# LANL-Bioinformatics/FaQCs

Hardware: AMD Instinct MI355X
Metric: M reads/sec (paired 2x150bp) (higher is better)
Workload: dtype u8; 1 GPU; synthetic 100M-pair 2x150bp Q33 reads resident in HBM per GPU, BWA_plus -q 5 --min_L 50, 1 step = 1 pass (trim_lds + counter all-reduce); pairs_per_gpu=100000000, read_len=150, terminal_n_supplied=True

## Files before the change

### faqcs_amd/csrc/faqcs_capi.hip

```cpp
#include "faqcs_ctx.h"

static uint8_t na_to_bits_host(char c)
{
    switch (c) {
    case 'A': case 'a': return 1;  case 'C': case 'c': return 2;  case 'G': case 'g': return 4;
    case 'T': case 't': return 8;  case 'M': case 'm': return 3;  case 'R': case 'r': return 5;
    case 'S': case 's': return 6;  case 'V': case 'v': return 7;  case 'W': case 'w': return 9;
    case 'Y': case 'y': return 10; case 'H': case 'h': return 11; case 'K': case 'k': return 12;
    case 'D': case 'd': return 13; case 'B': case 'b': return 14; case 'N': case 'n': return 15;
    case '-': return 16;
    }
    return 0;
}

static void build_avgq(const faqcs_params &p, std::vector<int32_t> &avgq)
{
    const int N = FAQCS_TAB_LEN + 1;
    avgq.assign(N, 0);
    const volatile float avg = p.average_quality;
    if (!(avg > 0.0f)) return;
    for (int len = 1; len < N; ++len) {
        auto pass = [&](int V) {
            volatile float t = (float)(V + p.input_quality_offset * len) / (float)len;
            volatile float v = t - (float)p.input_quality_offset;
// ... 69 lines not shown
    for (auto &rs : c->rec) { HIPCHK(hipEventCreateWithFlags(&rs.trimmed, hipEventDisableTiming)); HIPCHK(hipEventCreateWithFlags(&rs.folded, hipEventDisableTiming)); }
    HIPCHK(hipEventCreateWithFlags(&c->copied, hipEventDisableTiming));
    for (auto &sl : c->slot) HIPCHK(hipEventCreateWithFlags(&sl.done, hipEventDisableTiming));
    for (auto &e : c->ticket_ev) HIPCHK(hipEventCreateWithFlags(&e, hipEventDisableTiming));
    faqcs_counters_layout(p->max_read_length, p->n_adapters, &c->lay);

    std::vector<uint32_t> lcthr, magic, basetab; std::vector<int32_t> avgq; std::vector<float> norm;
    build_tables(*p, lcthr, avgq, norm, magic, basetab);
    HIPCHK(upload(&c->d_lcthr, lcthr)); HIPCHK(upload(&c->d_avgq, avgq)); HIPCHK(upload(&c->d_norm, norm));
    HIPCHK(upload(&c->d_magic, magic)); HIPCHK(upload(&c->d_basetab, basetab));
    HIPCHK(hipMalloc((void **)&c->d_counters, c->lay.total * sizeof(uint64_t)));
    HIPCHK(hipMemset(c->d_counters, 0, c->lay.total * sizeof(uint64_t)));
    HIPCHK(hipMalloc((void **)&c->d_err, 256));
    HIPCHK(hipMemset(c->d_err, 0, 256));
    {
        const size_t dwords = (size_t)c->n_cu * FAQCS_PARTIAL_FLUSHES * FAQCS_PARTIAL_ROW + (size_t)c->n_cu;
        HIPCHK(hipMalloc((void **)&c->d_partials, dwords * sizeof(uint32_t)));
        HIPCHK(hipMemset(c->d_partials, 0, dwords * sizeof(uint32_t)));
    }

    if (p->n_adapters) {
        std::vector<uint8_t> bits; std::vector<uint32_t> start(1, 0);
        for (uint32_t j = 0; j < p->n_adapters; ++j) {
            const char *s = p->adapter_seq[j];
            const size_t L = strlen(s);
            if (L == 0 || L > FAQCS_MAX_ADAPTER_LENGTH)
                return fail(FAQCS_E_INVAL, "faqcs_create: adapter " + std::to_string(j) + " has " + std::to_string(L) + " bases, 1 ... " +
                                               std::to_string(FAQCS_MAX_ADAPTER_LENGTH) + " are supported");
            c->adapters.emplace_back(s);
            for (size_t k = 0; k < L; ++k) {
                const uint8_t b = na_to_bits_host(s[k]);
                if (!b) return fail(FAQCS_E_BASE, "seq_overlap.cpp:na_to_bits: Unknown base!");
                bits.push_back(b);
// ... 31 lines not shown
            HIPCHK(upload(&c->d_awstart_grp, wgrp));
        }
    }

    DevParams &d = c->dp;
    memset(&d, 0, sizeof(d));
    d.mode = p->mode; d.Q = p->quality; d.in_off = p->input_quality_offset; d.out_off = p->output_quality_offset;
    auto cap16 = [](uint32_t v) { return v > 65535u ? 65535u : v; };
    d.min_len = cap16(p->min_read_length); d.max_poly_n = cap16(p->max_num_poly_N); d.trim5 = cap16(p->trim_5); d.trim3 = cap16(p->trim_3);
    d.replace_q = p->replace_to_N_q; d.protect5 = p->protect_5; d.qc_only = p->qc_only;
    d.has_adapters = p->n_adapters ? 1 : 0; d.avgq_on = p->average_quality > 0.0f ? 1 : 0;
    d.R = p->max_read_length; d.n_adapters = p->n_adapters;
    d.lc_ratio = p->low_complexity_cutoff_ratio; d.avg_q = p->average_quality;
    if (const char *e = getenv("FAQCS_DBG")) d.dbg = (uint32_t)strtoul(e, nullptr, 0);
    d.lc_thr = c->d_lcthr; d.avgq_min_v = c->d_avgq; d.comp_norm = c->d_norm; d.div_magic = c->d_magic; d.base_tab = c->d_basetab;
    d.partials = c->d_partials;
    d.partial_rows = c->d_partials + (size_t)c->n_cu * FAQCS_PARTIAL_FLUSHES * FAQCS_PARTIAL_ROW;
    d.lay = c->lay;

    c->kmer_active = p->kmer_rarefaction ? 1 : 0;
    if (p->kmer_rarefaction) {
        uint64_t slots = p->kmer_table_slots ? p->kmer_table_slots : (1ull << 28);
        uint64_t pow2 = 1; while (pow2 < slots) pow2 <<= 1;
        if (pow2 < (uint64_t)KG_SLICE_MIN << 16) pow2 = (uint64_t)KG_SLICE_MIN << 16;
        if (pow2 > (uint64_t)KG_SLICE_MAX << 16) return fail(FAQCS_E_INVAL, "faqcs_create: kmer_table_slots above 2^32");
        c->kt.mask = pow2 - 1;
        { uint32_t lg = 0; while ((1ull << lg) < pow2) ++lg; if (lg > 46) return fail(FAQCS_E_INVAL, "faqcs_create: kmer_table_slots too large"); c->kt.shift = 62 - lg; }
        if (const char *e = getenv("FAQCS_KMER_DIRECT")) c->kg.direct = atoi(e) != 0;
        c->kt.ovf_mask = std::max<uint64_t>(pow2 >> 4, 1ull << 16) - 1;
        { const uint32_t lg = 62 - c->kt.shift;
          int f = (int)lg - 27; f = f < 0 ? 0 : (f > 3 ? 3 : f);
          if (const char *e = getenv("FAQCS_KMER_FINE_BITS")) { const int v = atoi(e); if (v >= 0 && v <= 3) f = v; }
          while (f > 0 && (pow2 >> (16 + f)) < 16) --f;
// ... 15 lines not shown
extern "C" void faqcs_destroy(faqcs_ctx *c)
{
    if (!c) return;
    (void)hipSetDevice(c->device);
    if (c->compute) (void)hipStreamSynchronize(c->compute);
    if (c->copy) (void)hipStreamSynchronize(c->copy);
    if (c->aux) (void)hipStreamSynchronize(c->aux);
    for (auto &t : c->timings) { (void)hipEventDestroy(t.a); (void)hipEventDestroy(t.b); (void)hipEventDestroy(t.p); (void)hipEventDestroy(t.k0); (void)hipEventDestroy(t.k1); }
    if (c->comm) comm_release(c->comm);
    if (c->comm_ev) (void)hipEventDestroy(c->comm_ev);
    c->emit.release(); c->parse.release(); c->render.release(); c->pair.release(); c->render_pair.release(); c->inflate.release(); c->bgzf_index.release(); c->deflate.release(); c->detect.release(); c->gunzip.release();
    if (c->ins_a) (void)hipEventDestroy(c->ins_a);
    if (c->ins_b) (void)hipEventDestroy(c->ins_b);
    for (int k = 0; k < 2; ++k) { if (c->fwd_free[k]) (void)hipEventDestroy(c->fwd_free[k]); if (c->fwd_copied[k]) (void)hipEventDestroy(c->fwd_copied[k]); c->fwd_items[k].release(); }
    void *ptrs[] = {c->d_lcthr, c->d_basetab, c->d_avgq, c->d_norm, c->d_magic, c->d_counters, c->d_err, c->d_partials, c->d_abits, c->d_astart, c->d_aplanes, c->d_awstart,
                    c->d_awstart_grp, c->kt.slots, c->kt.stats, c->kt.dirty, c->d_fold_claim, c->d_snaps, c->d_ob, c->d_tot_by_epoch, c->d_first_hist};
    for (void *q : ptrs) if (q) (void)hipFree(q);
    for (auto &sl : c->slot) { sl.seq.release(); sl.qual.release(); sl.tn.release(); sl.off.release(); if (sl.done) (void)hipEventDestroy(sl.done); }
    for (auto &e : c->ticket_ev) if (e) (void)hipEventDestroy(e);
    c->s_seg.release(); c->s_sl.release(); c->s_hit.release(); c->s_res.release(); c->s_astate.release(); c->s_amask.release();
    for (auto &rs : c->rec) { rs.pre.release(); rs.post.release(); if (rs.trimmed) (void)hipEventDestroy(rs.trimmed); if (rs.folded) (void)hipEventDestroy(rs.folded); }
    if (c->aux) (void)hipStreamDestroy(c->aux);
    c->ob_items.release(); c->ob_wave_count.release(); c->ob_wave_offset.release();
    { void *kg_ptrs[] = {c->kg.dev.l1, c->kg.dev.l2, c->kg.dev.cur1, c->kg.dev.cur2, c->kg.dev.run_epoch, c->kg.dev.first_hist, c->kg.dev.tot_by_epoch, c->kg.dev.dense, c->kg.dev.big, c->kg.dev.n_big, c->kg.dev.redo};
      for (void *q : kg_ptrs) if (q) (void)hipFree(q);
      c->kg.defer.release();
      c->ks.l1.release(); c->ks.spill.release(); c->ks.cur1.release(); c->ks.run_epoch.release(); c->ks.defer.release(); c->ks.scratch.release();
      for (auto &ev : c->kg.flush_ev) { (void)hipEventDestroy(ev.first); (void)hipEventDestroy(ev.second); } }
    if (c->copied) (void)hipEventDestroy(c->copied);
    if (c->compute) (void)hipStreamDestroy(c->compute);
    if (c->copy) (void)hipStreamDestroy(c->copy);
// ... 55 lines not shown
    G.mask_words = (s.max_len + 63) / 64;
    HIPCHK(c->s_astate.reserve(n)); HIPCHK(c->s_amask.reserve((size_t)n * G.mask_words));
    HIPCHK(hipMemsetAsync(c->s_astate.p, 0, (size_t)n * sizeof(uint4), c->compute));
    G.state = c->s_astate.p; G.mask = c->s_amask.p; G.gstart = c->d_astart;
    for (size_t k = 0; k < c->agroups.size(); ++k) {
        const faqcs_ctx::AdapterGroupHost &g = c->agroups[k];
        AdapterDev A{c->d_abits, c->d_astart + g.j0, c->d_aplanes + 4 * (size_t)g.w0, c->d_awstart_grp + g.j0 + k, g.n, c->match_rate,
                     g.longest, g.plane_dwords};
        G.j0 = g.j0; G.last = k + 1 == c->agroups.size() ? 1u : 0u;
        HIPCHK(launch(A, &G));
    }
    return 0;
}

static bool env_on(const char *name) { const char *e = getenv(name); return !e || atoi(e) != 0; }

static int enqueue_trim(faqcs_ctx *c, Timing &t, const Submission &s, const uint32_t *d_sl, const uint16_t *d_hit)
{
    const uint32_t n = s.n;
    HIPCHK(hipEventRecord(t.a, c->compute));
    const bool tail_on = env_on("FAQCS_TAIL_FOLD");
    const bool offer_fold = c->pending_fold >= 0 && !c->pending_wide && tail_on;
    DevParams dp = c->dp;
    dp.fold_n = offer_fold ? c->pending_n : 0u;
    static const bool lds_on = env_on("FAQCS_TRIM_LDS"), lds4_on = env_on("FAQCS_TRIM_LDS4"), lds16_on = env_on("FAQCS_TRIM_LDS16");
    const char *e_long = getenv("FAQCS_TRIM_LONG");
    const TrimPlan plan = trim_plan(trim_options(dp), s.max_len, n, c->n_cu, TrimSwitches{e_long && atoi(e_long) != 0, lds_on, lds4_on, lds16_on});
    const bool long_reads = plan.kernel == TrimKernel::trim_long;
    dp.wide_records = plan.wide_records;
    const int set = (int)(c->n_enqueued++ & 1);
    faqcs_ctx::RecSet &rs = c->rec[set];
    if (rs.used) { HIPCHK(hipStreamWaitEvent(c->compute, rs.folded, 0)); rs.used = false; }
    const size_t need = plan.records_needed;
    if (need > rs.pre.cap) { HIPCHK(hipStreamSynchronize(c->aux)); HIPCHK(hipStreamSynchronize(c->compute)); }
    HIPCHK(rs.pre.reserve(need)); HIPCHK(rs.post.reserve(need));
    if (offer_fold) {
        const faqcs_ctx::RecSet &ps = c->rec[c->pending_fold];
        if (!c->d_fold_claim) HIPCHK(hipMalloc((void **)&c->d_fold_claim, 8));
        HIPCHK(hipMemsetAsync(c->d_fold_claim, 0, 8, c->compute));
        dp.fold_pre = ps.pre.p; dp.fold_post = ps.post.p; dp.fold_claim = c->d_fold_claim;
        dp.fold_dst_pre = c->d_counters + c->lay.pre_comp; dp.fold_dst_post = c->d_counters + c->lay.post_comp;
    }
    const TrimArgs a{s.seq, s.qual, s.off, n, s.max_len, d_sl, d_hit, s.tn, s.res, rs.pre.p, rs.post.p, c->d_counters, c->d_err, c->n_cu, c->compute};
    HIPCHK(long_reads ? faqcs_launch_trim_long(plan, dp, a)
                      : plan.kernel == TrimKernel::trim_lds ? faqcs_launch_trim_lds(plan, dp, a) : faqcs_launch_trim_filter_accumulate(plan, dp, a));
    HIPCHK(hipEventRecord(t.b, c->compute));
    c->trim_kernel = trim_kernel_name(plan.kernel);
    if (c->pending_fold >= 0) {
        if (!plan.folds_tail) {
            faqcs_ctx::RecSet &ps = c->rec[c->pending_fold];
            HIPCHK(hipStreamWaitEvent(c->aux, ps.trimmed, 0));
            HIPCHK(faqcs_launch_composition(ps.pre.p, ps.post.p, c->pending_n, c->pending_wide, c->d_norm, c->d_counters + c->lay.pre_comp,
                                            c->d_counters + c->lay.post_comp, c->n_cu, c->aux));
            HIPCHK(hipEventRecord(ps.folded, c->aux));
            ps.used = true;
        }
        c->pending_fold = -1;
    }
    static const bool no_comp = [] { const char *e = getenv("FAQCS_DIAG_NO_COMPOSITION"); return e && atoi(e) != 0; }();
    if (!(c->dp.dbg & 1u) && !long_reads && !no_comp) {
        HIPCHK(hipEventRecord(rs.trimmed, c->compute));
// ... 121 lines not shown
    if (!d_results) { HIPCHK(c->s_res.reserve((size_t)n + 1)); d_results = c->s_res.p; }
    return enqueue(c, b->seq, b->qual, b->offset, n, max_len, b->segment_start, b->n_segments, d_results, b->terminal_n);
}

extern "C" int faqcs_terminal_n_flags(int device_id, const uint8_t *d_seq, const uint32_t *d_offset, uint32_t n_reads, uint8_t *d_flags)
{
    if (!d_seq || !d_offset || !d_flags) return fail(FAQCS_E_INVAL, "null argument");
    if (device_id >= 0) HIPCHK(hipSetDevice(device_id));
    HIPCHK(faqcs_launch_terminal_n_flags(d_seq, d_offset, n_reads, d_flags, nullptr));
    HIPCHK(hipDeviceSynchronize());
    return 0;
}

int fold_pending_now(faqcs_ctx *c)
{
    if (c->pending_fold < 0) return 0;
    faqcs_ctx::RecSet &ps = c->rec[c->pending_fold];
    HIPCHK(faqcs_launch_composition(ps.pre.p, ps.post.p, c->pending_n, c->pending_wide, c->d_norm, c->d_counters + c->lay.pre_comp,
                                    c->d_counters + c->lay.post_comp, c->n_cu, c->compute));
    c->pending_fold = -1;
    return 0;
}

extern "C" int faqcs_sync(faqcs_ctx *c)
{
    if (!c) return fail(FAQCS_E_INVAL, "null ctx");
    HIPCHK(hipSetDevice(c->device));
    HIPCHK(hipStreamSynchronize(c->copy));
    if (int rc = fold_pending_now(c)) return rc;
    HIPCHK(hipStreamSynchronize(c->compute));
// ... 56 lines not shown
}

extern "C" int faqcs_finish(faqcs_ctx *c, uint64_t *counters, uint64_t n_u64)
{
    if (!c || !counters || n_u64 < c->lay.total) return fail(FAQCS_E_INVAL, "faqcs_finish: counter buffer too small");
    if (int rc = faqcs_sync(c)) return rc;
    HIPCHK(hipMemcpy(counters, c->d_counters, c->lay.total * sizeof(uint64_t), hipMemcpyDeviceToHost));
    return 0;
}

extern "C" int faqcs_reset_counters(faqcs_ctx *c)
{
    if (!c) return fail(FAQCS_E_INVAL, "null ctx");
    HIPCHK(hipSetDevice(c->device));
    c->pending_fold = -1;
    HIPCHK(hipStreamSynchronize(c->aux));
    HIPCHK(hipMemsetAsync(c->d_counters, 0, c->lay.total * sizeof(uint64_t), c->compute));
    return 0;
}

static int synth_fill_impl(int device_id, uint8_t *d_seq, uint8_t *d_qual, uint32_t *d_offset, uint32_t n_reads, uint32_t L,
                           uint64_t seed, uint64_t first_read, float adapter_frac, uint64_t genome_len)
{
    if (device_id >= 0) HIPCHK(hipSetDevice(device_id));
    if ((uint64_t)n_reads * L + L > 0xffffffffull) return fail(FAQCS_E_INVAL, "faqcs_synth_fill: arena exceeds 32-bit offsets");
    const char *at = getenv("FAQCS_SYNTH_AT");
    HIPCHK(faqcs_launch_synth(d_seq, d_qual, d_offset, n_reads, L, seed, first_read, adapter_frac, genome_len, at ? (float)atof(at) : -1.0f, nullptr));
    HIPCHK(hipDeviceSynchronize());
    return 0;
}
// ... 47 lines not shown
```

### faqcs_amd/csrc/faqcs_ctx.h

```cpp
#pragma once
#include <hip/hip_runtime.h>

#include <algorithm>
#include <cmath>
#include <cstdio>
#include <cstdlib>
#include <cstring>
#include <map>
#include <memory>
#include <string>
#include <vector>

#include "faqcs_dev.h"
#include "faqcs_host.h"
#include "faqcs_kmer.h"
#include "faqcs_skm.h"

struct AdapterDev {
    const uint8_t *bits;
    const uint32_t *start, *planes, *wstart;
    uint32_t n_adapters;
    float match_rate;
    uint32_t longest, plane_dwords;
};
hipError_t faqcs_launch_trim_lds(const TrimPlan &plan, const DevParams &P, const TrimArgs &a);
hipError_t faqcs_launch_trim_filter_accumulate(const TrimPlan &plan, const DevParams &P, const TrimArgs &a);
hipError_t faqcs_launch_trim_long(const TrimPlan &plan, const DevParams &P, const TrimArgs &a);
hipError_t faqcs_launch_terminal_n_flags(const uint8_t *seq, const uint32_t *off, uint32_t n_reads, uint8_t *flags, hipStream_t st);
hipError_t faqcs_launch_composition(const unsigned long long *rec_pre, const unsigned long long *rec_post, uint32_t n, bool wide,
                                    const float *comp_norm, uint64_t *dst_pre, uint64_t *dst_post, int n_cu, hipStream_t st);
hipError_t faqcs_launch_adapter(const AdapterDev &A, const AdapterGroup *G, const uint8_t *seq, const uint32_t *off, uint32_t n_reads,
                                uint32_t max_len, const uint32_t *seg_start, uint32_t n_segments, uint32_t *ad_sl,
                                uint16_t *ad_hit, uint64_t *adapter_stats, uint32_t *err, uint32_t dbg, int n_cu, hipStream_t st);
hipError_t faqcs_launch_synth(uint8_t *d_seq, uint8_t *d_qual, uint32_t *d_offset, uint32_t n_reads, uint32_t L,
                              uint64_t seed, uint64_t first_read, float adapter_frac, uint64_t genome_len, float at_frac, hipStream_t st);

size_t faqcs_emit_scratch_bytes(uint32_t n_reads);
hipError_t faqcs_launch_emit_scan(const uint8_t *seq, const uint32_t *off, const uint8_t *tn, uint32_t n_reads, const faqcs_read_result *res,
                                  const uint8_t *keep, const faqcs_emit_out *out, void *scratch, hipStream_t st);
hipError_t faqcs_launch_emit_gather(const uint8_t *seq, const uint8_t *qual, uint32_t n_reads, const faqcs_emit_out *out, const void *scratch,
// ... 128 lines not shown
    PackStage parse;
    PackStage render;
    PackStage pair;
    PackStage render_pair;
    PackStage inflate;
    PackStage bgzf_index;
    PackStage deflate;
    GunzipStage gunzip;
    PackStage detect;
    struct RecSet { DevBuf<unsigned long long> pre, post; hipEvent_t trimmed = nullptr, folded = nullptr; bool used = false; };
    RecSet rec[2];
    uint64_t n_enqueued = 0;
    int pending_fold = -1;
    uint32_t pending_n = 0;
    bool pending_wide = false;
    uint32_t *d_fold_claim = nullptr;
    hipStream_t aux = nullptr;
    uint64_t total_number = 0;
    int kmer_active = 0;
    std::vector<faqcs_rarefaction> points;
    struct PendingPoint { size_t point_index; size_t snap_index; };
    std::vector<PendingPoint> pending;
    KmerTable kt{nullptr, 0, nullptr, 0};
    bool partitioned = false;
    uint32_t part_rank = 0, part_world = 1, n_epochs = 0;
    std::vector<uint32_t> seg_epoch;
    DevBuf<ulonglong2> ob_items;
    bool ob_fresh = false;
    DevBuf<uint32_t> ob_wave_count;
    DevBuf<unsigned long long> ob_wave_offset;
    unsigned long long *d_ob = nullptr;
// ... 62 lines not shown
```

### faqcs_amd/csrc/faqcs_dev.h

```cpp
#pragma once
#include <hip/hip_runtime.h>
#include <stdint.h>

#include "../../include/faqcs_mi.h"
#include "faqcs_trim_plan.h"

#define FAQCS_WAVE 64
#define FAQCS_TAB_LEN FAQCS_FAST_READ_LENGTH

struct DevParams {
    int32_t mode, Q, in_off, out_off;
    uint32_t min_len, max_poly_n, trim5, trim3, replace_q;
    uint32_t protect5, qc_only, has_adapters, avgq_on;
    uint32_t R;
    uint32_t n_adapters;
    uint32_t dbg;
    uint32_t wide_records;
    float lc_ratio, avg_q;
    const uint32_t *lc_thr;
    const int32_t  *avgq_min_v;
    const uint32_t *div_magic;
    const float    *comp_norm;
    const uint32_t *base_tab;
    uint32_t *partials;
    uint32_t *partial_rows;
    faqcs_layout lay;
    const unsigned long long *fold_pre, *fold_post;
    uint32_t fold_n;
    uint32_t *fold_claim;
    uint64_t *fold_dst_pre, *fold_dst_post;
};

#define FAQCS_ADAPTER_GROUP 64
#define FAQCS_ADAPTER_TPL_CAP 4096
#define FAQCS_ADAPTER_SINGLE_LENGTH 8192

struct AdapterGroup {
    uint4 *state;
    uint64_t *mask;
    const uint32_t *gstart;
    uint32_t j0;
    uint32_t mask_words;
    uint32_t last;
};

enum { FAQCS_PARTIAL_ROW = 16896 };

struct TrimArgs {
    const uint8_t *seq, *qual;
    const uint32_t *off;
    uint32_t n_reads, max_len;
    const uint32_t *ad_sl;
    const uint16_t *ad_hit;
    const uint8_t *tn_flags;
    faqcs_read_result *out;
    unsigned long long *rec_pre, *rec_post;
    uint64_t *counters;
    uint32_t *err;
    int n_cu;
    hipStream_t st;
// ... 211 lines not shown
```

### faqcs_amd/csrc/faqcs_trim_common.h

```cpp
#pragma once
#include "faqcs_dev.h"

#include <stdlib.h>

static inline hipError_t ensure_dynamic_lds(const void *kernel, size_t bytes, unsigned long long &done)
{
    int dev = 0;
    hipError_t e = hipGetDevice(&dev);
    if (e != hipSuccess) return e;
    const unsigned long long bit = 1ull << (dev & 63);
    if (__atomic_load_n(&done, __ATOMIC_ACQUIRE) & bit) return hipSuccess;
    e = hipFuncSetAttribute(kernel, hipFuncAttributeMaxDynamicSharedMemorySize, (int)bytes);
    if (e == hipSuccess) __atomic_fetch_or(&done, bit, __ATOMIC_RELEASE);
    return e;
}

namespace {

template <int D> struct __attribute__((packed, aligned(1))) PackedBytes { uint32_t w[D]; };

__device__ __forceinline__ int med3i(int x, int lo, int hi) { return x < lo ? lo : (x > hi ? hi : x); }

template <int C> __device__ __forceinline__ uint32_t range_mask(int lo, int hi, int pbase)
{
// ... 501 lines not shown
        }
        if (dirty) {
            __syncthreads();
            for (int d = tid; d < ND; d += NT) {
                const uint32_t v = tab[d];
                if (v) {
                    tab[d] = 0;
                    if (v & 0xffffu) atomicAdd((unsigned long long *)(dst + 2 * d), (unsigned long long)(v & 0xffffu));
                    if (v >> 16) atomicAdd((unsigned long long *)(dst + 2 * d + 1), (unsigned long long)(v >> 16));
                }
            }
            __syncthreads();
        }
    }
}
#endif
```

### faqcs_amd/csrc/faqcs_trim_lds_kernel.hip

```cpp
#include "faqcs_trim_common.h"

#include <stdlib.h>
#include <type_traits>

#ifndef FAQCS_LDS_SUM_UNROLL
#define FAQCS_LDS_SUM_UNROLL 4
#endif
#ifndef FAQCS_LDS_SA_UNROLL
#define FAQCS_LDS_SA_UNROLL 2
#endif

namespace {

typedef uint32_t LdsPair2 __attribute__((ext_vector_type(2)));
typedef const __attribute__((address_space(3))) LdsPair2 *lds_u2c_ptr;
typedef __attribute__((address_space(3))) uint8_t *lds_u8_mut;
typedef const __attribute__((address_space(3))) uint8_t *lds_u8_ptr;
struct __attribute__((packed, aligned(1))) U32u { uint32_t w; };
typedef const __attribute__((address_space(3))) U32u *lds_u32u_ptr;

__device__ __forceinline__ uint32_t lds_ld(uint32_t byte_offset) { return *(lds_u32_ptr)(size_t)byte_offset; }
__device__ __forceinline__ uint32_t lds_ld_any(uint32_t byte_offset)
{
    const uint32_t a4 = byte_offset & ~3u;
// ... 158 lines not shown
__device__ __noinline__ void flush_block_partial(uint32_t *smem, uint32_t *__restrict__ row, const int tid)
{
    using Cfg = RowCfg<C, LPR, lds_wq(C, LPR)>;
    constexpr int N4 = (Cfg::N_ZERO + 3) / 4;
    static_assert(N4 * 4 <= FAQCS_PARTIAL_ROW, "partial-sum row");
    __syncthreads();
    for (int i = tid; i < N4; i += NW * 64) {
        const uint4 v = reinterpret_cast<const uint4 *>(smem)[i];
        reinterpret_cast<uint4 *>(row)[i] = v;
        if (4 * i + 3 < Cfg::N_ZERO) reinterpret_cast<uint4 *>(smem)[i] = make_uint4(0u, 0u, 0u, 0u);
        else for (int k = 4 * i; k < Cfg::N_ZERO; ++k) smem[k] = 0u;
    }
    __syncthreads();
}

template <int C, int LPR>
__global__ __launch_bounds__(1024) void fold_partials(const uint32_t *__restrict__ partials, const uint32_t *__restrict__ rows_used, const uint32_t n_blocks,
                                                      uint64_t *__restrict__ counters, const faqcs_layout lay, uint32_t *__restrict__ g_next)
{
    using Cfg = RowCfg<C, LPR, lds_wq(C, LPR)>;
    constexpr int W = Cfg::W;
    constexpr int CQ = lds_cq(C, LPR), QSTRIDE = lds_qstride(C, LPR);
    if (blockIdx.x == 0 && threadIdx.x == 0) *g_next = 0u;
    __shared__ unsigned long long part[2][16][64];
    const int i = blockIdx.x * 64 + (threadIdx.x & 63);
    unsigned long long lo = 0, hi = 0;
    if (i < Cfg::N_ZERO) {
        const bool halves = i < Cfg::O_BQPRE;
        for (uint32_t b = threadIdx.x >> 6; b < n_blocks; b += 16) {
            const uint32_t cnt = rows_used[b];
            const uint32_t *row = partials + (size_t)b * FAQCS_PARTIAL_FLUSHES * FAQCS_PARTIAL_ROW + i;
            for (uint32_t k = 0; k < cnt; ++k) {
                const uint32_t x = row[(size_t)k * FAQCS_PARTIAL_ROW];
                if (halves) { lo += x & 0xffffu; hi += x >> 16; } else lo += x;
            }
        }
    }
    part[0][threadIdx.x >> 6][threadIdx.x & 63] = lo;
    part[1][threadIdx.x >> 6][threadIdx.x & 63] = hi;
    __syncthreads();
    if (threadIdx.x >= 64 || i >= Cfg::N_ZERO) return;
    lo = 0; hi = 0;
#pragma unroll
    for (int g = 0; g < 16; ++g) { lo += part[0][g][threadIdx.x]; hi += part[1][g][threadIdx.x]; }
    if (!(lo | hi)) return;
    const uint64_t filter_stats = lay.filter_stats, pre_read_qhist = lay.pre_read_qhist, pre_base_qhist = lay.pre_base_qhist,
                   post_read_qhist = lay.post_read_qhist, post_base_qhist = lay.post_base_qhist, pre_len_hist = lay.pre_len_hist,
                   post_len_hist = lay.post_len_hist, pre_qual = lay.pre_qual, post_qual = lay.post_qual, pre_base = lay.pre_base,
                   post_base = lay.post_base;
    const uint32_t R = lay.max_read_length;
    auto add = [&](uint64_t idx, unsigned long long v) { if (v) atomicAdd((unsigned long long *)(counters + idx), v); };
    if (i < Cfg::O_HB) {
        const uint32_t q = (uint32_t)(i - Cfg::O_HQ) / Cfg::WQ, cell = (uint32_t)(i - Cfg::O_HQ) % Cfg::WQ;
        const uint32_t p = QSTRIDE == CQ ? cell : ((cell % QSTRIDE < (uint32_t)CQ && cell / QSTRIDE < (uint32_t)LPR) ? cell / QSTRIDE * CQ + cell % QSTRIDE : R);
        if (p < R) { add(pre_qual + (uint64_t)p * FAQCS_NQ + q, lo); add(post_qual + (uint64_t)p * FAQCS_NQ + q, hi); }
    } else if (i < Cfg::O_LEN) {
        const uint32_t c = (uint32_t)(i - Cfg::O_HB) / W, p = (uint32_t)(i - Cfg::O_HB) % W;
        if (p < R) { add(pre_base + (uint64_t)p * FAQCS_NBASE + c, lo); add(post_base + (uint64_t)p * FAQCS_NBASE + c, hi); }
    } else if (i < Cfg::O_RQ) {
        const uint32_t l = (uint32_t)(i - Cfg::O_LEN);
        if (l <= R) { add(pre_len_hist + l, lo); add(post_len_hist + l, hi); }
    } else if (i < Cfg::O_BQPRE) {
        const uint32_t k = (uint32_t)(i - Cfg::O_RQ);
        if (k < FAQCS_NQ) { add(pre_read_qhist + k, lo); add(post_read_qhist + k, hi); }
    } else if (i < Cfg::O_BQPOST) {
        add(pre_base_qhist + (uint32_t)(i - Cfg::O_BQPRE), lo);
    } else if (i < Cfg::O_FS) {
        add(post_base_qhist + (uint32_t)(i - Cfg::O_BQPOST), lo);
    } else {
        const uint32_t k = (uint32_t)(i - Cfg::O_FS);
        if (k < FAQCS_NUM_STAT) add(filter_stats + k, lo);
    }
}

template <int C, int NW, bool WINDOWED, bool EXT, int LPR, int RPC>
__global__ __launch_bounds__(NW * 64, NW / 4) void trim_lds(
    const DevParams P, const uint8_t *__restrict__ seq, const uint8_t *__restrict__ qual,
    const uint32_t *__restrict__ off, const uint32_t n_reads, const uint32_t *__restrict__ ad_sl,
    const uint16_t *__restrict__ ad_hit, uint2 *__restrict__ out, unsigned long long *__restrict__ rec_pre,
    unsigned long long *__restrict__ rec_post, uint64_t *__restrict__ counters, uint32_t *__restrict__ err,
    const uint8_t *__restrict__ tn_flags)
{
    static_assert(LPR == 8 || (LPR == 16 && (C == 16 || C == 19)) || (LPR == 4 && (C == 13 || C == 19)), "lanes per read");
    using Cfg = RowCfg<C, LPR, lds_wq(C, LPR)>;
    static_assert(RPC <= 64 && (RPC * LPR) % 64 == 0, "reads per chunk: the same number for every row of LPR lanes");
    using T = LdsCfg<C, NW, LPR, RPC>;
    using RW = RowOps<LPR>;
// ... 52 lines not shown
    const uint32_t rot = ROT ? (uint32_t)((lane / LPR) & (T::NROT - 1)) : 0u;
    if (ROT) {
        for (int i = tid; i < T::NROT * (CQ + 1) * 8; i += NW * 64) {
            const int r_ = i / ((CQ + 1) * 8), vb_ = (i / 8) % (CQ + 1), k_ = i % 8;
            uint32_t w_ = 0;
            for (int b_ = 0; b_ < 4; ++b_)
                if (4 * k_ + b_ < CQ && (4 * k_ + b_ + r_) % CQ < vb_) w_ |= 0xffu << (8 * b_);
            smem[T::O_TBQ + i] = w_;
        }
    }
    uint32_t three = 3u, wx4 = (uint32_t)(Cfg::WQ * 4);
    asm volatile("" : "+v"(three), "+v"(wx4));
    if (tid == 0 && blockIdx.x == 0 && (uint32_t)(size_t)((lds_u32_ptr)smem) != 0u) atomicOr(err, 4u);
    const uint32_t total_chunks = (n_reads + RPC - 1) / RPC;
    const uint32_t n_groups = (total_chunks + NW - 1) / NW;
    uint32_t *g_next = err + 8;
    if (tid == 0) {
        smem[T::O_CTR] = (uint32_t)NW;
        smem[T::O_CTR + 1] = 0xffffffffu;
        smem[T::O_CTR + 4] = blockIdx.x;
        smem[T::O_CTR + 5] = 0xffffffffu; smem[T::O_CTR + 6] = 0xffffffffu; smem[T::O_CTR + 7] = 0xffffffffu;
        const uint32_t g1 = gridDim.x + atomicAdd(g_next, 1u);
        if (g1 < n_groups) smem[T::O_CTR + 5] = (1u << 20) | g1; else smem[T::O_CTR + 1] = (uint32_t)NW;
    }
    __syncthreads();

    constexpr uint32_t FLUSH_CHUNKS = lds_flush_chunks(NW, RPC);
    constexpr uint32_t MAX_GROUPS = (uint32_t)FAQCS_PARTIAL_FLUSHES * FLUSH_CHUNKS / NW;
    constexpr uint32_t REG_FLUSH_EVERY = 63 / TPR;
    constexpr uint32_t NO_CHUNK = 0xffffffffu;
    auto lds_word = [&](const int i) { return uniu(*(volatile const __attribute__((address_space(3))) uint32_t *)(size_t)(uint32_t)((T::O_CTR + i) * 4)); };
// ... 943 lines not shown
            oc.N = pN | (cN << 16);
            oc.Vpre = V_pre; oc.Vpost = V_post;

            chunk_epilogue<LPR>(oc, mine, my, v_len, v_hit, lane, smem + Cfg::O_LEN, smem + Cfg::O_RQ, smem + Cfg::O_BQPRE,
                                smem + Cfg::O_BQPOST, smem + Cfg::O_FS, smem + Cfg::O_TMAGIC, out, rec_pre, rec_post, EXT && P.avgq_on != 0, 0u, &fs_acc,
                                WIDE && P.wide_records != 0u, true);
            ld = ld_next;
            }
        }

        FAQCS_STAMP(8)
        c_cur = c_next; chunk_cur = chunk_next;
    }
    if (__any((any_err & 1u) != 0) && lane == 0) atomicOr(err, 1u);
    if (tid == 0) P.partial_rows[blockIdx.x] = n_flushed;
    if (lds_tail_folds_v<C, NW, LPR, RPC> && P.fold_n) {
        __syncthreads();
        comp_fold_tail<NW * 64>(smem, P, tid, blockIdx.x & 1u);
    }
#ifdef FAQCS_LDS_STAMPS
    if (lane == 0) {
#pragma unroll
        for (int i = 0; i < 9; ++i) atomicAdd(reinterpret_cast<unsigned long long *>(err + 16) + i, st_acc[i]);
        atomicAdd(reinterpret_cast<unsigned long long *>(err + 16) + 9, __builtin_amdgcn_s_memtime() - clk0);
        atomicAdd(reinterpret_cast<unsigned long long *>(err + 16) + 11, st_flush);
#ifdef FAQCS_LDS_BLOCKLOG
        if (wave == 0) printf("block %u xcc %u chunks %u start %llu end %llu\n", blockIdx.x, __builtin_amdgcn_s_getreg((20 << 0) | (0 << 6) | (3 << 11)), smem[T::O_CTR + 1],
                              (unsigned long long)rt0, (unsigned long long)__builtin_amdgcn_s_memrealtime());
#endif
        if (wave == 0) {
// ... 25 lines not shown
}

template <int C, bool WINDOWED, bool EXT, int LPR = 8, int RPC = 64>
static hipError_t launch_trim_lds(const TrimPlan &plan, const DevParams &P, const TrimArgs &a)
{
    constexpr int NW = lds_waves(C, LPR, RPC);
    constexpr size_t lds = (size_t)LdsCfg<C, NW, LPR, RPC>::lds_dwords() * 4;
    static unsigned long long attr_done = 0;
    auto kern = trim_lds<C, NW, WINDOWED, EXT, LPR, RPC>;
    if (plan.NW != NW || plan.RPC != RPC) return hipErrorInvalidValue;
    if (hipError_t e = ensure_dynamic_lds(reinterpret_cast<const void *>(kern), lds, attr_done); e != hipSuccess) return e;
    if (plan.grid == 0) return hipSuccess;
    hipLaunchKernelGGL(kern, dim3(plan.grid), dim3(NW * 64), lds, a.st, P, a.seq, a.qual, a.off, a.n_reads, a.ad_sl, a.ad_hit,
                       reinterpret_cast<uint2 *>(a.out), a.rec_pre, a.rec_post, a.counters, a.err, a.tn_flags);
    if (hipError_t e = hipGetLastError(); e != hipSuccess) return e;
    hipLaunchKernelGGL((fold_partials<C, LPR>), dim3((RowCfg<C, LPR, lds_wq(C, LPR)>::N_ZERO + 63) / 64), dim3(1024), 0, a.st, P.partials, P.partial_rows, plan.grid, a.counters, P.lay, a.err + 8);
    return hipGetLastError();
}

using TrimLaunch = hipError_t (*)(const TrimPlan &, const DevParams &, const TrimArgs &);
template <int C, int LPR, int RPC> static TrimLaunch trim_lds_variant(const TrimPlan &plan)
{
    return plan.ext ? (plan.windowed ? launch_trim_lds<C, true, true, LPR, RPC> : launch_trim_lds<C, false, true, LPR, RPC>)
                    : (plan.windowed ? launch_trim_lds<C, true, false, LPR, RPC> : launch_trim_lds<C, false, false, LPR, RPC>);
}

hipError_t faqcs_launch_trim_lds(const TrimPlan &plan, const DevParams &P, const TrimArgs &a)
{
    TrimLaunch f = nullptr;
    switch (trim_shape_key(plan.C, plan.LPR)) {
    case trim_shape_key(13, 4): f = trim_lds_variant<13, 4, 64>(plan); break;
    case trim_shape_key(19, 4): f = trim_lds_variant<19, 4, 64>(plan); break;
    case trim_shape_key(13, 8): f = trim_lds_variant<13, 8, 64>(plan); break;
    case trim_shape_key(19, 8): f = trim_lds_variant<19, 8, 64>(plan); break;
    case trim_shape_key(16, 16): f = trim_lds_variant<16, 16, FAQCS_LDS16_RPC>(plan); break;
    case trim_shape_key(19, 16): f = trim_lds_variant<19, 16, 20>(plan); break;
    }
    return f ? f(plan, P, a) : hipErrorInvalidValue;
}
```

Measured before the change: 9470 M reads/s.

## Defer partial-row fold into next trim_lds launch tail with double-buffered partials

Removes the separate fold_partials launch after each trim_lds pass. Partial rows now go into one of two alternating buffers, and the next trim_lds launch folds the previous launch's partials in its tail using an atomic slice-claim counter. If no further LDS launch follows, a standalone fold kernel runs at flush time, and that kernel now splits the block range across four CTAs per slice with an unrolled reduction. The cost is twice the partials memory, a control word block in device memory, and more fold work inside the trim kernel tail, which may add registers or latency.

```diff
diff --git a/faqcs_amd/csrc/faqcs_capi.hip b/faqcs_amd/csrc/faqcs_capi.hip
--- a/faqcs_amd/csrc/faqcs_capi.hip
+++ b/faqcs_amd/csrc/faqcs_capi.hip
@@ -107,9 +107,13 @@
     HIPCHK(hipMalloc((void **)&c->d_err, 256));
     HIPCHK(hipMemset(c->d_err, 0, 256));
     {
-        const size_t dwords = (size_t)c->n_cu * FAQCS_PARTIAL_FLUSHES * FAQCS_PARTIAL_ROW + (size_t)c->n_cu;
+        const size_t dwords = 2 * c->partial_set_dwords();
         HIPCHK(hipMalloc((void **)&c->d_partials, dwords * sizeof(uint32_t)));
         HIPCHK(hipMemset(c->d_partials, 0, dwords * sizeof(uint32_t)));
+        static_assert(2 * FAQCS_CTL_WORDS * sizeof(uint32_t) <= 64, "the layout's copy starts 64 bytes into d_ctl");
+        HIPCHK(hipMalloc((void **)&c->d_ctl, 64 + sizeof(faqcs_layout)));
+        HIPCHK(hipMemset(c->d_ctl, 0, 64));
+        HIPCHK(hipMemcpy(reinterpret_cast<uint8_t *>(c->d_ctl) + 64, &c->lay, sizeof(faqcs_layout), hipMemcpyHostToDevice));
     }
 
     if (p->n_adapters) {
@@ -171,9 +175,8 @@
     d.lc_ratio = p->low_complexity_cutoff_ratio; d.avg_q = p->average_quality;
     if (const char *e = getenv("FAQCS_DBG")) d.dbg = (uint32_t)strtoul(e, nullptr, 0);
     d.lc_thr = c->d_lcthr; d.avgq_min_v = c->d_avgq; d.comp_norm = c->d_norm; d.div_magic = c->d_magic; d.base_tab = c->d_basetab;
-    d.partials = c->d_partials;
-    d.partial_rows = c->d_partials + (size_t)c->n_cu * FAQCS_PARTIAL_FLUSHES * FAQCS_PARTIAL_ROW;
     d.lay = c->lay;
+    d.lay_dev = reinterpret_cast<const faqcs_layout *>(reinterpret_cast<const uint8_t *>(c->d_ctl) + 64);
 
     c->kmer_active = p->kmer_rarefaction ? 1 : 0;
     if (p->kmer_rarefaction) {
@@ -219,7 +222,7 @@
     if (c->ins_b) (void)hipEventDestroy(c->ins_b);
     for (int k = 0; k < 2; ++k) { if (c->fwd_free[k]) (void)hipEventDestroy(c->fwd_free[k]); if (c->fwd_copied[k]) (void)hipEventDestroy(c->fwd_copied[k]); c->fwd_items[k].release(); }
     void *ptrs[] = {c->d_lcthr, c->d_basetab, c->d_avgq, c->d_norm, c->d_magic, c->d_counters, c->d_err, c->d_partials, c->d_abits, c->d_astart, c->d_aplanes, c->d_awstart,
-                    c->d_awstart_grp, c->kt.slots, c->kt.stats, c->kt.dirty, c->d_fold_claim, c->d_snaps, c->d_ob, c->d_tot_by_epoch, c->d_first_hist};
+                    c->d_awstart_grp, c->kt.slots, c->kt.stats, c->kt.dirty, c->d_ctl, c->d_snaps, c->d_ob, c->d_tot_by_epoch, c->d_first_hist};
     for (void *q : ptrs) if (q) (void)hipFree(q);
     for (auto &sl : c->slot) { sl.seq.release(); sl.qual.release(); sl.tn.release(); sl.off.release(); if (sl.done) (void)hipEventDestroy(sl.done); }
     for (auto &e : c->ticket_ev) if (e) (void)hipEventDestroy(e);
@@ -305,6 +308,15 @@
 }
 
 static bool env_on(const char *name) { const char *e = getenv(name); return !e || atoi(e) != 0; }
+
+static int fold_rows_now(faqcs_ctx *c)
+{
+    if (!c->rows_pending) return 0;
+    HIPCHK(faqcs_launch_fold_partials(c->rows_C, c->rows_LPR, c->partial_set(c->rows_set), c->partial_set_rows(c->rows_set), c->rows_grid, c->d_counters,
+                                      c->lay, c->compute));
+    c->rows_pending = false;
+    return 0;
+}
 
 static int enqueue_trim(faqcs_ctx *c, Timing &t, const Submission &s, const uint32_t *d_sl, const uint16_t *d_hit)
 {
@@ -325,17 +337,29 @@
     const size_t need = plan.records_needed;
     if (need > rs.pre.cap) { HIPCHK(hipStreamSynchronize(c->aux)); HIPCHK(hipStreamSynchronize(c->compute)); }
     HIPCHK(rs.pre.reserve(need)); HIPCHK(rs.post.reserve(need));
+    const bool lds = plan.kernel == TrimKernel::trim_lds && plan.grid > 0;
+    if (c->rows_pending && !(lds && tail_on && plan.C == c->rows_C && plan.LPR == c->rows_LPR)) { if (int rc = fold_rows_now(c)) return rc; }
+    const int lset = (int)(c->n_lds_launches & 1);
+    if (lds) {
+        dp.partials = c->partial_set(lset); dp.partial_rows = c->partial_set_rows(lset);
+        dp.ctl = c->d_ctl + lset * FAQCS_CTL_WORDS; dp.ctl_other = c->d_ctl + (lset ^ 1) * FAQCS_CTL_WORDS;
+        if (c->rows_pending) {
+            dp.prev_partials = c->partial_set(c->rows_set); dp.prev_rows = c->partial_set_rows(c->rows_set); dp.prev_grid = c->rows_grid;
+        }
+    }
     if (offer_fold) {
         const faqcs_ctx::RecSet &ps = c->rec[c->pending_fold];
-        if (!c->d_fold_claim) HIPCHK(hipMalloc((void **)&c->d_fold_claim, 8));
-        HIPCHK(hipMemsetAsync(c->d_fold_claim, 0, 8, c->compute));
-        dp.fold_pre = ps.pre.p; dp.fold_post = ps.post.p; dp.fold_claim = c->d_fold_claim;
+        dp.fold_pre = ps.pre.p; dp.fold_post = ps.post.p; dp.fold_claim = dp.ctl ? dp.ctl + FAQCS_CTL_FOLD : nullptr;
         dp.fold_dst_pre = c->d_counters + c->lay.pre_comp; dp.fold_dst_post = c->d_counters + c->lay.post_comp;
     }
     const TrimArgs a{s.seq, s.qual, s.off, n, s.max_len, d_sl, d_hit, s.tn, s.res, rs.pre.p, rs.post.p, c->d_counters, c->d_err, c->n_cu, c->compute};
     HIPCHK(long_reads ? faqcs_launch_trim_long(plan, dp, a)
                       : plan.kernel == TrimKernel::trim_lds ? faqcs_launch_trim_lds(plan, dp, a) : faqcs_launch_trim_filter_accumulate(plan, dp, a));
     HIPCHK(hipEventRecord(t.b, c->compute));
+    if (lds) {
+        c->rows_pending = true; c->rows_set = lset; c->rows_C = plan.C; c->rows_LPR = plan.LPR; c->rows_grid = plan.grid;
+        ++c->n_lds_launches;
+    }
     c->trim_kernel = trim_kernel_name(plan.kernel);
     if (c->pending_fold >= 0) {
         if (!plan.folds_tail) {
@@ -487,6 +511,7 @@
 
 int fold_pending_now(faqcs_ctx *c)
 {
+    if (int rc = fold_rows_now(c)) return rc;
     if (c->pending_fold < 0) return 0;
     faqcs_ctx::RecSet &ps = c->rec[c->pending_fold];
     HIPCHK(faqcs_launch_composition(ps.pre.p, ps.post.p, c->pending_n, c->pending_wide, c->d_norm, c->d_counters + c->lay.pre_comp,
@@ -573,6 +598,7 @@
     if (!c) return fail(FAQCS_E_INVAL, "null ctx");
     HIPCHK(hipSetDevice(c->device));
     c->pending_fold = -1;
+    c->rows_pending = false;
     HIPCHK(hipStreamSynchronize(c->aux));
     HIPCHK(hipMemsetAsync(c->d_counters, 0, c->lay.total * sizeof(uint64_t), c->compute));
     return 0;
diff --git a/faqcs_amd/csrc/faqcs_ctx.h b/faqcs_amd/csrc/faqcs_ctx.h
--- a/faqcs_amd/csrc/faqcs_ctx.h
+++ b/faqcs_amd/csrc/faqcs_ctx.h
@@ -24,6 +24,8 @@
     uint32_t longest, plane_dwords;
 };
 hipError_t faqcs_launch_trim_lds(const TrimPlan &plan, const DevParams &P, const TrimArgs &a);
+hipError_t faqcs_launch_fold_partials(int C, int LPR, const uint32_t *partials, const uint32_t *rows_used, uint32_t grid, uint64_t *counters,
+                                      const faqcs_layout &lay, hipStream_t st);
 hipError_t faqcs_launch_trim_filter_accumulate(const TrimPlan &plan, const DevParams &P, const TrimArgs &a);
 hipError_t faqcs_launch_trim_long(const TrimPlan &plan, const DevParams &P, const TrimArgs &a);
 hipError_t faqcs_launch_terminal_n_flags(const uint8_t *seq, const uint32_t *off, uint32_t n_reads, uint8_t *flags, hipStream_t st);
@@ -182,7 +184,14 @@
     int pending_fold = -1;
     uint32_t pending_n = 0;
     bool pending_wide = false;
-    uint32_t *d_fold_claim = nullptr;
+    uint64_t n_lds_launches = 0;
+    bool rows_pending = false;
+    int rows_set = 0, rows_C = 0, rows_LPR = 0;
+    uint32_t rows_grid = 0;
+    uint32_t *d_ctl = nullptr;
+    size_t partial_set_dwords() const { return ((size_t)n_cu * FAQCS_PARTIAL_FLUSHES * FAQCS_PARTIAL_ROW + (size_t)n_cu + 3) & ~(size_t)3; }
+    uint32_t *partial_set(int set) const { return d_partials + (size_t)set * partial_set_dwords(); }
+    uint32_t *partial_set_rows(int set) const { return partial_set(set) + (size_t)n_cu * FAQCS_PARTIAL_FLUSHES * FAQCS_PARTIAL_ROW; }
     hipStream_t aux = nullptr;
     uint64_t total_number = 0;
     int kmer_active = 0;
diff --git a/faqcs_amd/csrc/faqcs_dev.h b/faqcs_amd/csrc/faqcs_dev.h
--- a/faqcs_amd/csrc/faqcs_dev.h
+++ b/faqcs_amd/csrc/faqcs_dev.h
@@ -24,7 +24,11 @@
     const uint32_t *base_tab;
     uint32_t *partials;
     uint32_t *partial_rows;
+    const uint32_t *prev_partials, *prev_rows;
+    uint32_t prev_grid;
+    uint32_t *ctl, *ctl_other;
     faqcs_layout lay;
+    const faqcs_layout *lay_dev;
     const unsigned long long *fold_pre, *fold_post;
     uint32_t fold_n;
     uint32_t *fold_claim;
@@ -44,6 +48,7 @@
     uint32_t last;
 };
 
+enum { FAQCS_CTL_GROUP = 0, FAQCS_CTL_FOLD = 1, FAQCS_CTL_ROWS = 3, FAQCS_CTL_WORDS = 4 };
 enum { FAQCS_PARTIAL_ROW = 16896 };
 
 struct TrimArgs {
diff --git a/faqcs_amd/csrc/faqcs_trim_common.h b/faqcs_amd/csrc/faqcs_trim_common.h
--- a/faqcs_amd/csrc/faqcs_trim_common.h
+++ b/faqcs_amd/csrc/faqcs_trim_common.h
@@ -539,4 +539,97 @@
         }
     }
 }
+
+template <int C, int LPR>
+__device__ __forceinline__ void partials_cell_add(const int i, const unsigned long long lo, const unsigned long long hi, uint64_t *__restrict__ counters,
+                                                  const faqcs_layout &lay)
+{
+    using Cfg = RowCfg<C, LPR, lds_wq(C, LPR)>;
+    constexpr int W = Cfg::W;
+    constexpr int CQ = lds_cq(C, LPR), QSTRIDE = lds_qstride(C, LPR);
+    const uint32_t R = lay.max_read_length;
+    auto add = [&](uint64_t idx, unsigned long long v) { if (v) atomicAdd((unsigned long long *)(counters + idx), v); };
+    if (i < Cfg::O_HB) {
+        const uint32_t q = (uint32_t)(i - Cfg::O_HQ) / Cfg::WQ, cell = (uint32_t)(i - Cfg::O_HQ) % Cfg::WQ;
+        const uint32_t p = QSTRIDE == CQ ? cell : ((cell % QSTRIDE < (uint32_t)CQ && cell / QSTRIDE < (uint32_t)LPR) ? cell / QSTRIDE * CQ + cell % QSTRIDE : R);
+        if (p < R) { add(lay.pre_qual + (uint64_t)p * FAQCS_NQ + q, lo); add(lay.post_qual + (uint64_t)p * FAQCS_NQ + q, hi); }
+    } else if (i < Cfg::O_LEN) {
+        const uint32_t c = (uint32_t)(i - Cfg::O_HB) / W, p = (uint32_t)(i - Cfg::O_HB) % W;
+        if (p < R) { add(lay.pre_base + (uint64_t)p * FAQCS_NBASE + c, lo); add(lay.post_base + (uint64_t)p * FAQCS_NBASE + c, hi); }
+    } else if (i < Cfg::O_RQ) {
+        const uint32_t l = (uint32_t)(i - Cfg::O_LEN);
+        if (l <= R) { add(lay.pre_len_hist + l, lo); add(lay.post_len_hist + l, hi); }
+    } else if (i < Cfg::O_BQPRE) {
+        const uint32_t k = (uint32_t)(i - Cfg::O_RQ);
+        if (k < FAQCS_NQ) { add(lay.pre_read_qhist + k, lo); add(lay.post_read_qhist + k, hi); }
+    } else if (i < Cfg::O_BQPOST) {
+        add(lay.pre_base_qhist + (uint32_t)(i - Cfg::O_BQPRE), lo);
+    } else if (i < Cfg::O_FS) {
+        add(lay.post_base_qhist + (uint32_t)(i - Cfg::O_BQPOST), lo);
+    } else if (i < Cfg::N_ZERO) {
+        const uint32_t k = (uint32_t)(i - Cfg::O_FS);
+        if (k < FAQCS_NUM_STAT) add(lay.filter_stats + k, lo);
+    }
+}
+template <int C, int LPR>
+__device__ __forceinline__ void partial_rows_sum(const uint32_t *__restrict__ partials, const uint32_t *__restrict__ rows_used, const uint32_t n_blocks,
+                                                 const int i, const uint32_t b0, const uint32_t bstep, unsigned long long &lo, unsigned long long &hi)
+{
+    using Cfg = RowCfg<C, LPR, lds_wq(C, LPR)>;
+    constexpr int U = 4;
+    constexpr size_t BLOCK_DW = (size_t)FAQCS_PARTIAL_FLUSHES * FAQCS_PARTIAL_ROW;
+    const bool halves = i < Cfg::O_BQPRE;
+    auto acc = [&](const uint32_t x) { if (halves) { lo += x & 0xffffu; hi += x >> 16; } else lo += x; };
+    for (uint32_t b = b0; b < n_blocks; b += U * bstep) {
+        uint32_t cnt[U], x0[U], x1[U];
+#pragma unroll
+        for (int u = 0; u < U; ++u) {
+            const uint32_t bb = b + (uint32_t)u * bstep;
+            cnt[u] = bb < n_blocks ? umin_(rows_used[bb], (uint32_t)FAQCS_PARTIAL_FLUSHES) : 0u;
+        }
+#pragma unroll
+        for (int u = 0; u < U; ++u) {
+            const uint32_t *row = partials + (size_t)(b + (uint32_t)u * bstep) * BLOCK_DW + i;
+            x0[u] = cnt[u] > 0u ? row[0] : 0u;
+            x1[u] = cnt[u] > 1u ? row[FAQCS_PARTIAL_ROW] : 0u;
+        }
+#pragma unroll
+        for (int u = 0; u < U; ++u) { acc(x0[u]); acc(x1[u]); }
+#pragma unroll
+        for (int u = 0; u < U; ++u) {
+            const uint32_t *row = partials + (size_t)(b + (uint32_t)u * bstep) * BLOCK_DW + i;
+            for (uint32_t k = 2; k < cnt[u]; ++k) acc(row[(size_t)k * FAQCS_PARTIAL_ROW]);
+        }
+    }
+}
+template <int C, int LPR, int NW>
+__device__ __noinline__ void partials_fold_tail(uint32_t *smem, const uint32_t *__restrict__ prev, const uint32_t *__restrict__ prev_rows, const uint32_t prev_grid,
+                                                uint32_t *__restrict__ claim, uint64_t *__restrict__ counters, const faqcs_layout *__restrict__ lay_dev, const int tid)
+{
+    using Cfg = RowCfg<C, LPR, lds_wq(C, LPR)>;
+    constexpr uint32_t N_SLICES = (Cfg::N_ZERO + 63) / 64;
+    unsigned long long *part = reinterpret_cast<unsigned long long *>(smem);
+    uint32_t *s_next = smem + 2 * NW * 64 * 2;
+    const int lane = tid & 63, wave = tid >> 6;
+    __syncthreads();
+#pragma unroll 1
+    for (;;) {
+        if (tid == 0) *s_next = atomicAdd(claim, 1u);
+        __syncthreads();
+        const uint32_t s = *s_next;
+        if (s >= N_SLICES) return;
+        const int i = (int)(s * 64u) + lane;
+        unsigned long long lo = 0, hi = 0;
+        if (i < Cfg::N_ZERO) partial_rows_sum<C, LPR>(prev, prev_rows, prev_grid, i, (uint32_t)wave, (uint32_t)NW, lo, hi);
+        part[wave * 64 + lane] = lo;
+        part[(NW + wave) * 64 + lane] = hi;
+        __syncthreads();
+        if (wave == 0) {
+            lo = 0; hi = 0;
+#pragma unroll
+            for (int g = 0; g < NW; ++g) { lo += part[g * 64 + lane]; hi += part[(NW + g) * 64 + lane]; }
+            if (lo | hi) partials_cell_add<C, LPR>(i, lo, hi, counters, *lay_dev);
+        }
+    }
+}
 #endif
diff --git a/faqcs_amd/csrc/faqcs_trim_lds_kernel.hip b/faqcs_amd/csrc/faqcs_trim_lds_kernel.hip
--- a/faqcs_amd/csrc/faqcs_trim_lds_kernel.hip
+++ b/faqcs_amd/csrc/faqcs_trim_lds_kernel.hip
@@ -196,28 +196,17 @@
     __syncthreads();
 }
 
+enum { FOLD_SPLIT = 4 };
 template <int C, int LPR>
 __global__ __launch_bounds__(1024) void fold_partials(const uint32_t *__restrict__ partials, const uint32_t *__restrict__ rows_used, const uint32_t n_blocks,
-                                                      uint64_t *__restrict__ counters, const faqcs_layout lay, uint32_t *__restrict__ g_next)
+                                                      uint64_t *__restrict__ counters, const faqcs_layout lay)
 {
     using Cfg = RowCfg<C, LPR, lds_wq(C, LPR)>;
-    constexpr int W = Cfg::W;
-    constexpr int CQ = lds_cq(C, LPR), QSTRIDE = lds_qstride(C, LPR);
-    if (blockIdx.x == 0 && threadIdx.x == 0) *g_next = 0u;
     __shared__ unsigned long long part[2][16][64];
-    const int i = blockIdx.x * 64 + (threadIdx.x & 63);
+    const int i = (int)(blockIdx.x / FOLD_SPLIT) * 64 + (int)(threadIdx.x & 63);
+    const uint32_t set = (blockIdx.x % FOLD_SPLIT) * 16u + (threadIdx.x >> 6);
     unsigned long long lo = 0, hi = 0;
-    if (i < Cfg::N_ZERO) {
-        const bool halves = i < Cfg::O_BQPRE;
-        for (uint32_t b = threadIdx.x >> 6; b < n_blocks; b += 16) {
-            const uint32_t cnt = rows_used[b];
-            const uint32_t *row = partials + (size_t)b * FAQCS_PARTIAL_FLUSHES * FAQCS_PARTIAL_ROW + i;
-            for (uint32_t k = 0; k < cnt; ++k) {
-                const uint32_t x = row[(size_t)k * FAQCS_PARTIAL_ROW];
-                if (halves) { lo += x & 0xffffu; hi += x >> 16; } else lo += x;
-            }
-        }
-    }
+    if (i < Cfg::N_ZERO) partial_rows_sum<C, LPR>(partials, rows_used, n_blocks, i, set, 16u * FOLD_SPLIT, lo, hi);
     part[0][threadIdx.x >> 6][threadIdx.x & 63] = lo;
     part[1][threadIdx.x >> 6][threadIdx.x & 63] = hi;
     __syncthreads();
@@ -225,34 +214,7 @@
     lo = 0; hi = 0;
 #pragma unroll
     for (int g = 0; g < 16; ++g) { lo += part[0][g][threadIdx.x]; hi += part[1][g][threadIdx.x]; }
-    if (!(lo | hi)) return;
-    const uint64_t filter_stats = lay.filter_stats, pre_read_qhist = lay.pre_read_qhist, pre_base_qhist = lay.pre_base_qhist,
-                   post_read_qhist = lay.post_read_qhist, post_base_qhist = lay.post_base_qhist, pre_len_hist = lay.pre_len_hist,
-                   post_len_hist = lay.post_len_hist, pre_qual = lay.pre_qual, post_qual = lay.post_qual, pre_base = lay.pre_base,
-                   post_base = lay.post_base;
-    const uint32_t R = lay.max_read_length;
-    auto add = [&](uint64_t idx, unsigned long long v) { if (v) atomicAdd((unsigned long long *)(counters + idx), v); };
-    if (i < Cfg::O_HB) {
-        const uint32_t q = (uint32_t)(i - Cfg::O_HQ) / Cfg::WQ, cell = (uint32_t)(i - Cfg::O_HQ) % Cfg::WQ;
-        const uint32_t p = QSTRIDE == CQ ? cell : ((cell % QSTRIDE < (uint32_t)CQ && cell / QSTRIDE < (uint32_t)LPR) ? cell / QSTRIDE * CQ + cell % QSTRIDE : R);
-        if (p < R) { add(pre_qual + (uint64_t)p * FAQCS_NQ + q, lo); add(post_qual + (uint64_t)p * FAQCS_NQ + q, hi); }
-    } else if (i < Cfg::O_LEN) {
-        const uint32_t c = (uint32_t)(i - Cfg::O_HB) / W, p = (uint32_t)(i - Cfg::O_HB) % W;
-        if (p < R) { add(pre_base + (uint64_t)p * FAQCS_NBASE + c, lo); add(post_base + (uint64_t)p * FAQCS_NBASE + c, hi); }
-    } else if (i < Cfg::O_RQ) {
-        const uint32_t l = (uint32_t)(i - Cfg::O_LEN);
-        if (l <= R) { add(pre_len_hist + l, lo); add(post_len_hist + l, hi); }
-    } else if (i < Cfg::O_BQPRE) {
-        const uint32_t k = (uint32_t)(i - Cfg::O_RQ);
-        if (k < FAQCS_NQ) { add(pre_read_qhist + k, lo); add(post_read_qhist + k, hi); }
-    } else if (i < Cfg::O_BQPOST) {
-        add(pre_base_qhist + (uint32_t)(i - Cfg::O_BQPRE), lo);
-    } else if (i < Cfg::O_FS) {
-        add(post_base_qhist + (uint32_t)(i - Cfg::O_BQPOST), lo);
-    } else {
-        const uint32_t k = (uint32_t)(i - Cfg::O_FS);
-        if (k < FAQCS_NUM_STAT) add(filter_stats + k, lo);
-    }
+    if (lo | hi) partials_cell_add<C, LPR>(i, lo, hi, counters, lay);
 }
 
 template <int C, int NW, bool WINDOWED, bool EXT, int LPR, int RPC>
@@ -335,7 +297,11 @@
     if (tid == 0 && blockIdx.x == 0 && (uint32_t)(size_t)((lds_u32_ptr)smem) != 0u) atomicOr(err, 4u);
     const uint32_t total_chunks = (n_reads + RPC - 1) / RPC;
     const uint32_t n_groups = (total_chunks + NW - 1) / NW;
-    uint32_t *g_next = err + 8;
+    uint32_t *g_next = P.ctl + FAQCS_CTL_GROUP;
+    if (tid == 0 && blockIdx.x == 0) {
+#pragma unroll
+        for (int i = 0; i < FAQCS_CTL_WORDS; ++i) P.ctl_other[i] = 0u;
+    }
     if (tid == 0) {
         smem[T::O_CTR] = (uint32_t)NW;
         smem[T::O_CTR + 1] = 0xffffffffu;
@@ -1309,6 +1275,11 @@
     }
     if (__any((any_err & 1u) != 0) && lane == 0) atomicOr(err, 1u);
     if (tid == 0) P.partial_rows[blockIdx.x] = n_flushed;
+    {
+        const __attribute__((address_space(4))) DevParams *Pk = (const __attribute__((address_space(4))) DevParams *)__builtin_amdgcn_kernarg_segment_ptr();
+        const uint32_t prev_grid = Pk->prev_grid;
+        if (prev_grid) partials_fold_tail<C, LPR, NW>(smem, Pk->prev_partials, Pk->prev_rows, prev_grid, Pk->ctl + FAQCS_CTL_ROWS, counters, Pk->lay_dev, tid);
+    }
     if (lds_tail_folds_v<C, NW, LPR, RPC> && P.fold_n) {
         __syncthreads();
         comp_fold_tail<NW * 64>(smem, P, tid, blockIdx.x & 1u);
@@ -1364,7 +1335,6 @@
     hipLaunchKernelGGL(kern, dim3(plan.grid), dim3(NW * 64), lds, a.st, P, a.seq, a.qual, a.off, a.n_reads, a.ad_sl, a.ad_hit,
                        reinterpret_cast<uint2 *>(a.out), a.rec_pre, a.rec_post, a.counters, a.err, a.tn_flags);
     if (hipError_t e = hipGetLastError(); e != hipSuccess) return e;
-    hipLaunchKernelGGL((fold_partials<C, LPR>), dim3((RowCfg<C, LPR, lds_wq(C, LPR)>::N_ZERO + 63) / 64), dim3(1024), 0, a.st, P.partials, P.partial_rows, plan.grid, a.counters, P.lay, a.err + 8);
     return hipGetLastError();
 }
 
@@ -1388,3 +1358,25 @@
     }
     return f ? f(plan, P, a) : hipErrorInvalidValue;
 }
+
+template <int C, int LPR>
+static hipError_t launch_fold_partials(const uint32_t *partials, const uint32_t *rows_used, uint32_t grid, uint64_t *counters, const faqcs_layout &lay, hipStream_t st)
+{
+    constexpr int slices = (RowCfg<C, LPR, lds_wq(C, LPR)>::N_ZERO + 63) / 64;
+    hipLaunchKernelGGL((fold_partials<C, LPR>), dim3(slices * FOLD_SPLIT), dim3(1024), 0, st, partials, rows_used, grid, counters, lay);
+    return hipGetLastError();
+}
+hipError_t faqcs_launch_fold_partials(int C, int LPR, const uint32_t *partials, const uint32_t *rows_used, uint32_t grid, uint64_t *counters,
+                                      const faqcs_layout &lay, hipStream_t st)
+{
+    if (!grid) return hipSuccess;
+    switch (trim_shape_key(C, LPR)) {
+    case trim_shape_key(13, 4): return launch_fold_partials<13, 4>(partials, rows_used, grid, counters, lay, st);
+    case trim_shape_key(19, 4): return launch_fold_partials<19, 4>(partials, rows_used, grid, counters, lay, st);
+    case trim_shape_key(13, 8): return launch_fold_partials<13, 8>(partials, rows_used, grid, counters, lay, st);
+    case trim_shape_key(19, 8): return launch_fold_partials<19, 8>(partials, rows_used, grid, counters, lay, st);
+    case trim_shape_key(16, 16): return launch_fold_partials<16, 16>(partials, rows_used, grid, counters, lay, st);
+    case trim_shape_key(19, 16): return launch_fold_partials<19, 16>(partials, rows_used, grid, counters, lay, st);
+    }
+    return hipErrorInvalidValue;
+}
```

Result: no change. 9518 M reads/s, median of 6 (+0.5%).
